# broadinstitute/Tangram

Hardware: NVIDIA H100
Metric: map_cells_to_space iterations/sec (higher is better)
Workload: dtype bf16 operands / f32 accumulate+state

## Files before the change

### tangram_b200/csrc/adam_rows.cuh

```cuda
#pragma once
#include "common.cuh"
#include "gemm_tc.cuh"

namespace tgb {

struct AdamRowsArgs {
  float* M; __nv_bfloat16* m; float* v;
  const __nv_bfloat16* dq;
  __nv_bfloat16* Pt;
  const RowConst* rowc;
  float* zsum; float* pxsum; float* l1sum; float* l2sum;
  int ld, V, row0, row1;
  float lam_r, lam_l1, lam_l2;
  AdamScalars a;
};

__device__ __forceinline__ void ldg256f(const float* src, float (&x)[8]) {
  asm volatile("ld.global.cs.v4.f32 {%0,%1,%2,%3}, [%8];\n\t"
               "ld.global.cs.v4.f32 {%4,%5,%6,%7}, [%8+16];"
               : "=f"(x[0]), "=f"(x[1]), "=f"(x[2]), "=f"(x[3]), "=f"(x[4]), "=f"(x[5]), "=f"(x[6]), "=f"(x[7]) : "l"(src));
}
__device__ __forceinline__ void stg256f(float* dst, const float (&x)[8]) {
  asm volatile("st.global.cs.v4.f32 [%0], {%1,%2,%3,%4};\n\t"
               "st.global.cs.v4.f32 [%0+16], {%5,%6,%7,%8};"
               ::"l"(dst), "f"(x[0]), "f"(x[1]), "f"(x[2]), "f"(x[3]), "f"(x[4]), "f"(x[5]), "f"(x[6]), "f"(x[7]) : "memory");
}
__device__ __forceinline__ uint4 ldg128_stream(const void* src) {
  uint4 r;
  asm volatile("ld.global.nc.L1::no_allocate.v4.b32 {%0,%1,%2,%3}, [%4];" : "=r"(r.x), "=r"(r.y), "=r"(r.z), "=r"(r.w) : "l"(src));
  return r;
}

struct AdamRowsLoad { float x[8], m[8], v[8]; uint4 d, mq; };

__device__ __forceinline__ void unpack_bf8(const uint4& q, float (&f)[8]) {
  const uint32_t w[4] = {q.x, q.y, q.z, q.w};
#pragma unroll
  for (int e = 0; e < 4; ++e) {
    const __nv_bfloat162 b = *reinterpret_cast<const __nv_bfloat162*>(&w[e]);
    f[2 * e] = __low2float(b); f[2 * e + 1] = __high2float(b);
  }
}
__device__ __forceinline__ uint4 pack_bf8(const float (&f)[8]) {
  uint4 o;
  __nv_bfloat162 b;
  b = __floats2bfloat162_rn(f[0], f[1]); o.x = *reinterpret_cast<uint32_t*>(&b);
  b = __floats2bfloat162_rn(f[2], f[3]); o.y = *reinterpret_cast<uint32_t*>(&b);
  b = __floats2bfloat162_rn(f[4], f[5]); o.z = *reinterpret_cast<uint32_t*>(&b);
  b = __floats2bfloat162_rn(f[6], f[7]); o.w = *reinterpret_cast<uint32_t*>(&b);
  return o;
}

#ifndef TGB_ADAM_MAXNREG
#define TGB_ADAM_MAXNREG 96
#endif
template <bool PLAIN>
__global__ void __maxnreg__(TGB_ADAM_MAXNREG)
k_adam_rows(const AdamRowsArgs p) {
  const int lane = threadIdx.x & 31;
  const int row = p.row0 + blockIdx.x * 8 + (threadIdx.x >> 5);
  if (row >= p.row1) return;
  const RowConst rc = p.rowc[row];
  const float lse_l2e = rc.lse * 1.4426950408889634f;
  const size_t base = (size_t)row * p.ld;
  float* Mr = p.M + base; __nv_bfloat16* mr = p.m + base; float* vr = p.v + base;
  const __nv_bfloat16* dr = p.dq + base;
  __nv_bfloat16* pr = p.Pt + base;

  const float k_nstep = -p.a.step_size;

  float zs = 0.f, pxs = 0.f, l1s = 0.f, l2s = 0.f;

  auto load = [&](int c, AdamRowsLoad& L) {
    ldg256f(Mr + c, L.x); L.mq = ldg128_stream(mr + c); ldg256f(vr + c, L.v);
    L.d = ldg128_stream(dr + c);
  };
  auto one = [&](float& x, float dq, float& m, float& v) -> float {
    const float pcur = fast_ex2(fmaf(x, 1.4426950408889634f, -lse_l2e));
    float g = dq - rc.r;
    if (p.lam_r != 0.f) g -= p.lam_r * ((x - rc.lse) - rc.h);
    g *= pcur;
    if (p.lam_l1 != 0.f) g += p.lam_l1 * (float)((x > 0.f) - (x < 0.f));
    if (p.lam_l2 != 0.f) g += 2.f * p.lam_l2 * x;
    m = fmaf(g - m, p.a.one_minus_beta1, m);
    v = fmaf(p.a.one_minus_beta2 * g, g, v * p.a.beta2);
    const float denom = fmaf(fast_sqrt(v), p.a.inv_bc2_sqrt, p.a.eps);
    x = fmaf(-p.a.step_size * m, fast_rcp(denom), x);
    const float pt = fast_ex2(fmaf(x, 1.4426950408889634f, -lse_l2e));
    zs += pt;
    if (p.pxsum) pxs = fmaf(pt, x, pxs);
    if (p.l1sum) { l1s += fabsf(x); l2s = fmaf(x, x, l2s); }
    return pt;
  };
  auto process = [&](int c, AdamRowsLoad& L) {
// ... 33 lines not shown
        const float dq = (e & 1) ? __high2float(d2) : __low2float(d2);
        pt[e] = (c + e < p.V) ? one(L.x[e], dq, L.m[e], L.v[e]) : 0.f;
      }
      stg256f(Mr + c, L.x); *reinterpret_cast<uint4*>(mr + c) = pack_bf8(L.m); stg256f(vr + c, L.v);
    } else {
#pragma unroll
      for (int e = 0; e < 8; ++e) pt[e] = 0.f;
    }
    *reinterpret_cast<uint4*>(pr + c) = pack_bf8(pt);
  };

  int c = lane * 8;
  for (; c + 256 < p.ld; c += 512) {
    AdamRowsLoad A, B;
    load(c, A);
    load(c + 256, B);
    process(c, A);
    process(c + 256, B);
  }
  if (c < p.ld) {
    AdamRowsLoad A;
    load(c, A);
    process(c, A);
  }
  zs = warp_sum(zs);
  if (p.pxsum) pxs = warp_sum(pxs);
  if (p.l1sum) { l1s = warp_sum(l1s); l2s = warp_sum(l2s); }
  if (lane == 0) {
    p.zsum[row] = zs;
    if (p.pxsum) p.pxsum[row] = pxs;
    if (p.l1sum) { p.l1sum[row] = l1s; p.l2sum[row] = l2s; }
  }
}

struct AdamRowsExactArgs {
  float* M; float* m; float* v;
  const float* dp;
  const RowStat* stats; const float* rdot;
  int ld, V, row0, row1;
  float lam_r, lam_l1, lam_l2;
  AdamScalars a;
};

__global__ void __launch_bounds__(256)
k_adam_rows_exact(const AdamRowsExactArgs p) {
  const int lane = threadIdx.x & 31;
  const int row = p.row0 + blockIdx.x * 8 + (threadIdx.x >> 5);
  if (row >= p.row1) return;
  const RowStat st = p.stats[row];
  const float r = p.rdot[row];
  const size_t base = (size_t)row * p.ld;
  float* Mr = p.M + base; float* mr = p.m + base; float* vr = p.v + base;
  const float* dr = p.dp + base;
  for (int c = lane * 8; c < p.V; c += 256) {
    float x[8], m[8], v[8], d[8];
    ldg256f(Mr + c, x); ldg256f(mr + c, m); ldg256f(vr + c, v); ldg256f(dr + c, d);
#pragma unroll
    for (int e = 0; e < 8; ++e) {
      if (c + e < p.V) {
        const float pr = softmax_prob(x[e], st);
        float g = d[e] - r;
        if (p.lam_r != 0.f) g -= p.lam_r * (((x[e] - st.mx) - st.log_z) - st.h);
        g *= pr;
        if (p.lam_l1 != 0.f) g += p.lam_l1 * (float)((x[e] > 0.f) - (x[e] < 0.f));
        if (p.lam_l2 != 0.f) g += 2.f * p.lam_l2 * x[e];
        x[e] = adam_update(x[e], g, m[e], v[e], p.a);
// ... 25 lines not shown
```

### tangram_b200/csrc/gemm_tc.cuh

```cuda
#pragma once
#include <cuda.h>
#include <cstdio>
#include "common.cuh"
#include "gemm_simt.cuh"

namespace tgb {

constexpr int TC_BM = 128;
constexpr int TC_BK = 64;
constexpr int TC_MMA_K = 16;
constexpr int TC_BN = 256;
constexpr int TC_THREADS = 384;
constexpr int TC_ACC = TC_BN / 2;

__device__ __forceinline__ uint32_t smem_u32(const void* p) { return (uint32_t)__cvta_generic_to_shared(p); }

__device__ __forceinline__ void mbar_init(uint64_t* bar, uint32_t count) {
  asm volatile("mbarrier.init.shared::cta.b64 [%0], %1;" ::"r"(smem_u32(bar)), "r"(count));
}
__device__ __forceinline__ void mbar_expect_tx(uint64_t* bar, uint32_t bytes) {
  asm volatile("mbarrier.arrive.expect_tx.shared::cta.b64 _, [%0], %1;" ::"r"(smem_u32(bar)), "r"(bytes) : "memory");
}
__device__ __forceinline__ void mbar_wait(uint64_t* bar, uint32_t parity) {
  asm volatile(
// ... 460 lines not shown
static inline int tc_init(TcContext& tc, char* err, size_t n) {
  void* fn = nullptr;
  cudaDriverEntryPointQueryResult qres;
  cudaError_t e = cudaGetDriverEntryPoint("cuTensorMapEncodeTiled", &fn, cudaEnableDefault, &qres);
  if (e != cudaSuccess || fn == nullptr || qres != cudaDriverEntryPointSuccess) {
    snprintf(err, n, "cuTensorMapEncodeTiled not available from the driver (%s)", cudaGetErrorString(e));
    return -2;
  }
  tc.encode = (PFN_encodeTiled)fn;
  int dev = 0;
  cudaGetDevice(&dev);
  cudaDeviceGetAttribute(&tc.num_sms, cudaDevAttrMultiProcessorCount, dev);
  return 0;
}

static inline int tc_make_map(TcContext& tc, CUtensorMap* map, const void* base, uint64_t cols, uint64_t rows,
                              uint64_t ld, uint32_t box_inner, uint32_t box_outer, char* err, size_t n) {
  cuuint64_t dims[2] = {cols, rows};
  cuuint64_t strides[1] = {ld * 2};
  cuuint32_t box[2] = {box_inner, box_outer};
  cuuint32_t estr[2] = {1, 1};
  CUresult r = tc.encode(map, CU_TENSOR_MAP_DATA_TYPE_BFLOAT16, 2, const_cast<void*>(base), dims, strides, box, estr,
                         CU_TENSOR_MAP_INTERLEAVE_NONE, CU_TENSOR_MAP_SWIZZLE_128B, CU_TENSOR_MAP_L2_PROMOTION_L2_256B,
                         CU_TENSOR_MAP_FLOAT_OOB_FILL_NONE);
  if (r != CUDA_SUCCESS) {
    snprintf(err, n, "cuTensorMapEncodeTiled failed (%d) cols=%llu rows=%llu ld=%llu box=%ux%u", (int)r,
             (unsigned long long)cols, (unsigned long long)rows, (unsigned long long)ld, box_inner, box_outer);
    return -2;
  }
  return 0;
}

template <class Kern, class... Args>
static inline int tc_launch(TcContext& tc, Kern kern, int smem, long long pairs, cudaStream_t s, const char* name, char* err,
                            size_t n, Args... args) {
  cudaLaunchAttribute attr[1];
  attr[0].id = cudaLaunchAttributeClusterDimension;
  attr[0].val.clusterDim.x = 2;
  attr[0].val.clusterDim.y = 1;
  attr[0].val.clusterDim.z = 1;
  cudaLaunchConfig_t cfg = {};
  cfg.blockDim = dim3(TC_THREADS);
  cfg.dynamicSmemBytes = (size_t)smem;
  cfg.stream = s;
  cfg.attrs = attr;
  cfg.numAttrs = 1;
  const void* key = reinterpret_cast<const void*>(kern);
  int slot = -1;
  for (int i = 0; i < 16; ++i) {
    if (tc.smem_fn[i] == key) { slot = i; break; }
    if (tc.smem_fn[i] == nullptr && slot < 0) slot = i;
  }
  if (slot < 0) { snprintf(err, n, "launch %s: more than 16 tensor-core kernels", name); return -2; }
  if (tc.smem_fn[slot] != key || tc.smem_bytes[slot] != smem) {
    cudaError_t e = cudaFuncSetAttribute(kern, cudaFuncAttributeMaxDynamicSharedMemorySize, smem);
    if (e != cudaSuccess) { snprintf(err, n, "cudaFuncSetAttribute(smem=%d): %s", smem, cudaGetErrorString(e)); return -2; }
    cfg.gridDim = dim3(2);
    int c = 0;
    e = cudaOccupancyMaxActiveClusters(&c, kern, &cfg);
    if (e != cudaSuccess || c < 1) {
      snprintf(err, n, "launch %s: no 2-CTA cluster with %d B of shared memory fits (%s)", name, smem, cudaGetErrorString(e));
      return -2;
    }
    tc.smem_fn[slot] = key; tc.smem_bytes[slot] = smem; tc.clusters[slot] = c;
  }
  cfg.gridDim = dim3((unsigned)(2 * (pairs < tc.clusters[slot] ? pairs : tc.clusters[slot])));
  cudaError_t e = cudaLaunchKernelEx(&cfg, kern, args...);
  if (e == cudaSuccess) e = cudaGetLastError();
  if (e != cudaSuccess) { snprintf(err, n, "launch %s: %s", name, cudaGetErrorString(e)); return -2; }
  return 0;
}

constexpr int TC_STAGE_BYTES = (TC_BM + TC_BN) * TC_BK * 2;
constexpr int TC_SMEM_LIMIT = 227 * 1024;
template <class Epi>
constexpr int tc_stages() {
  const int fit = (TC_SMEM_LIMIT - 2048 - Epi::kSmemBytes) / TC_STAGE_BYTES;
  return fit < 4 ? fit : 4;
}
template <class Epi>
constexpr int tc_smem() { return tc_stages<Epi>() * TC_STAGE_BYTES + Epi::kSmemBytes + 1024; }
constexpr int TC_SMEM = tc_smem<TcEpiStore>();
static inline int tc_dp_row_parts(int V) { return (int)ceil_div(V, TC_BN); }
static inline int tc_splits(int num_sms, long long tiles, long long k_total, int min_k) {
  long long s = (2LL * num_sms + tiles - 1) / tiles;
  const long long max_s = (k_total + min_k - 1) / min_k;
  if (s > max_s) s = max_s;
  if (s < 1) s = 1;
  const long long kps = ((k_total + s - 1) / s + TC_BK - 1) / TC_BK * TC_BK;
  return (int)((k_total + kps - 1) / kps);
}
static inline int tc_splits_for_chain(long long k_total, int max_chain) {
  long long s = (k_total + max_chain - 1) / max_chain;
  if (s < 1) s = 1;
  const long long kps = ((k_total + s - 1) / s + TC_BK - 1) / TC_BK * TC_BK;
  return (int)((k_total + kps - 1) / kps);
}
static inline int tc_forward_splits(int num_sms, int N, int V, int Ke) {
  return tc_splits(num_sms, (long long)ceil_div(V, TC_BM) * ceil_div(Ke, TC_BN), N, 512);
}
static inline int tc_kps(int k_total, int splits) {
  return (int)(round_up(ceil_div(k_total, splits), TC_BK));
}
static inline long long tc_pairs(int tiles_m, int tiles_n, int splits) { return (long long)(tiles_m + 1) / 2 * tiles_n * splits; }

static inline int tc_make_maps(TcContext& tc, TcMaps* maps, const __nv_bfloat16* base, size_t plane_elems, int n_planes,
                               uint64_t cols, uint64_t rows, uint64_t ld, uint32_t bi, uint32_t bo, char* err, size_t n) {
  for (int p = 0; p < 3; ++p) {
    const __nv_bfloat16* ptr = base + (size_t)(p < n_planes ? p : 0) * plane_elems;
    if (tc_make_map(tc, &maps->m[p], ptr, cols, rows, ld, bi, bo, err, n)) return -2;
  }
  return 0;
}

struct TcPlan {
  TcMaps a, b;
  CUtensorMap pt, dq;
  bool ready = false;
};

static inline int tc_forward_plan(TcContext& tc, TcPlan& pl, const __nv_bfloat16* P, size_t p_plane, const __nv_bfloat16* Sx,
                                  size_t s_plane, int planes, int N, int V, int Ke, int ld, char* err, size_t n) {
  if (tc_make_maps(tc, &pl.a, P, p_plane, planes, V, N, ld, 64, 64, err, n)) return -2;
  if (tc_make_maps(tc, &pl.b, Sx, s_plane, planes, Ke, N, Ke, 64, 64, err, n)) return -2;
  pl.ready = true;
  return 0;
}
static inline int tc_forward_launch(TcContext& tc, const TcPlan& pl, int n_pairs, float* out, int N, int V, int Ke, int splits,
                                    cudaStream_t s, char* err, size_t n) {
  auto kern = k_gemm_tc<false, false, tc_stages<TcEpiStore>(), TcEpiStore>;
  TcEpiStore epi{out, Ke, (size_t)V * Ke, V, 0};
  const int tm = (int)ceil_div(V, TC_BM), tn = (int)ceil_div(Ke, TC_BN);
  return tc_launch(tc, kern, TC_SMEM, tc_pairs(tm, tn, splits), s, "tc_gemm_fwd", err, n, pl.a, pl.b, n_pairs, N, tc_kps(N, splits),
                   tm, tn, splits, 1, kPolicyEvictNormal, kPolicyEvictNormal, 0, 0, epi);
}
static inline int tc_forward_launch_rows(TcContext& tc, const TcPlan& pl, int n_pairs, float* out, int accumulate, int row0, int row1,
                                         int V, int Ke, cudaStream_t s, char* err, size_t n) {
  auto kern = k_gemm_tc<false, false, tc_stages<TcEpiStore>(), TcEpiStore>;
  TcEpiStore epi{out, Ke, (size_t)V * Ke, V, accumulate};
  const int tm = (int)ceil_div(V, TC_BM), tn = (int)ceil_div(Ke, TC_BN);
  return tc_launch(tc, kern, TC_SMEM, tc_pairs(tm, tn, 1), s, "tc_gemm_fwd", err, n, pl.a, pl.b, n_pairs, row1,
                   (int)round_up(row1 - row0, TC_BK), tm, tn, 1, 1, kPolicyEvictNormal, kPolicyEvictNormal, 0, row0, epi);
}

static inline int tc_dpstore_plan(TcContext& tc, TcPlan& pl, const __nv_bfloat16* Sxb, size_t s_plane, const __nv_bfloat16* dYb,
                                  size_t dy_plane, int planes, int N, int V, int Ke, char* err, size_t n) {
  if (tc_make_maps(tc, &pl.a, Sxb, s_plane, planes, Ke, N, Ke, 64, TC_BM, err, n)) return -2;
  if (tc_make_maps(tc, &pl.b, dYb, dy_plane, planes, Ke, V, Ke, 64, TC_BN / 2, err, n)) return -2;
  pl.ready = true;
  return 0;
}
static inline int tc_dpstore_epi_plan(TcContext& tc, TcPlan& pl, const __nv_bfloat16* Pt, const __nv_bfloat16* dq, int N, int ld,
                                      char* err, size_t n) {
  if (tc_make_map(tc, &pl.pt, Pt, ld, N, ld, 64, 64, err, n)) return -2;
  return tc_make_map(tc, &pl.dq, dq, ld, N, ld, 64, 64, err, n);
}
template <class Epi>
static inline int tc_dpstore_launch(TcContext& tc, const TcPlan& pl, int n_pairs, const Epi& epi, int row0, int row1, int V, int Ke,
                                    cudaStream_t s, char* err, size_t n) {
  const int tn = (int)ceil_div(V, TC_BN);
  auto kern = k_gemm_tc<true, true, tc_stages<Epi>(), Epi>;
  constexpr int smem = tc_smem<Epi>();
  const int tm0 = row0 / TC_BM, tm = (int)ceil_div(row1, TC_BM) - tm0;
  return tc_launch(tc, kern, smem, tc_pairs(tm, tn, 1), s, "tc_gemm_bwd_dp", err, n, pl.a, pl.b, n_pairs, Ke, Ke, tm, tn, 1, 1,
                   kPolicyEvictNormal, kPolicyEvictLast, tm0, 0, epi);
}

}
```

### tangram_b200/csrc/tangram_b200.cu

```cuda
#include "../../include/tangram_b200.h"

#include <algorithm>
#include <cmath>
#include <cstdarg>
#include <cstdio>
#include <cstdlib>
#include <cstring>
#include <mutex>
#include <string>
#include <thread>
#include <vector>

#include "common.cuh"
#include "kernels_elem.cuh"
#include "gemm_simt.cuh"
#include "gemm_tc.cuh"
#include "adam_rows.cuh"
#include "legacy_rng.cuh"
#include "agreement.cuh"
#include "annotate.cuh"
#include "project.cuh"
#include "group_stats.cuh"
#include "mt19937_jump.h"
#include "nccl_dl.h"
// ... 97 lines not shown
  int fwd_splits = 1;
  DevBuf<float> Ypart;
  DevBuf<float> Y;
  DevBuf<float> dY;
  DevBuf<__nv_bfloat16> dYb;
  DevBuf<float> ngc, ngr, WG, nwg, AG, nag, sgnG, Z, Zg, H;
  DevBuf<float> colpart, colpart_nb, colpart_go, rowpart, ctpart;
  DevBuf<float> coefA, coefB, coefAn, coefBn, coefAg, coefBg, coefAr, coefBr, densg;
  CsrDev W, WT, F, FT, A, AT;
  int nchunk = 0, ncolchunk = 0, nredchunk = 0, n_ct_blocks = 0, loss_rows = 16;
  DevBuf<float> colfin;
  bool masked = false;
  int n_active = 0;
  DevBuf<float> gene_act;
  DevBuf<float> gw;
  int val_every = 0;
  int64_t val_epoch = 0;
  int64_t val_row = -1;
  bool tail_stale = false;
  DevBuf<float> val_coef, val_rowpart, val_hist;
  DevBuf<float> hist;
  int64_t hist_len = 0, hist_cap = 0;
  bool have_expr = false, have_density = false, have_ct = false, have_mapping = false;
  bool in_step = false;
  int64_t launches = 0;
  float legacy_stats[8] = {0};
  TcContext tc;
  TcPlan plan_fwd, plan_dp;
  DevBuf<__nv_bfloat16> dq;
  DevBuf<__nv_bfloat16> mb;
  DevBuf<float> rcenter;
  DevBuf<float> dpf;
  bool pipelined = false;
  bool host_state = false;
  int R = 0;
  int ring_rows = 0;
  DevBuf<float> Mh, mh, vh;
  DevBuf<__nv_bfloat16> mbh;
  DevBuf<float> rM[2], rm[2], rv[2];
  DevBuf<__nv_bfloat16> rmb[2];
  cudaStream_t cin = nullptr, cout = nullptr;
  cudaEvent_t ev_in[2] = {}, ev_comp[2] = {}, ev_free[2] = {}, ev_start = nullptr, ev_last = nullptr;
  bool ring_used = false;
  int nchunks = 1, chunk_row[9] = {0};
  cudaStream_t hi = nullptr, lo = nullptr, sf = nullptr;
  cudaEvent_t ev_fork = nullptr, ev_join_hi = nullptr, ev_join_lo = nullptr, ev_join_sf = nullptr, ev_loss = nullptr;
  cudaEvent_t ev_g[8] = {}, ev_a[8] = {}, ev_f[8] = {};
  bool a_valid = false;
  bool fwd_ahead = false;
  bool recording = false;
  std::vector<LaunchRecord> records;
  void drop_records(size_t from) {
    for (size_t i = from; i < records.size(); ++i) cudaEventDestroy(records[i].ev);
    records.resize(from);
  }
  void* comm = nullptr;
  bool comm_owned = false;
  int comm_rank = 0, comm_world = 1;
  bool y_nccl = false;
  void* y_reg = nullptr;
  void release_exchange_registration() {
    if (!y_nccl) return;
    char e[64];
    if (NcclApi* a = nccl_api(e, sizeof(e))) {
      if (y_reg && comm) a->CommDeregister(comm, y_reg);
      a->MemFree(Y.p);
// ... 275 lines not shown
  } else {
    A(h->Pf.alloc(nv));
  }
  A(h->Sx.alloc((size_t)h->N * h->Ke));
  A(h->G.alloc(vk));
  A(h->d.alloc(h->V)); A(h->dsrc.alloc(h->N));
  A(h->stats.alloc(h->N)); A(h->rowaux.alloc((size_t)2 * h->N)); A(h->rdot.alloc(h->N));
  int nc = 1;
  if (h->bf16) {
    nc = h->N >= 32768 ? 4 : (h->N >= 8192 ? 2 : 1);
    if (const char* e = getenv("TGB200_CHUNKS")) nc = atoi(e);
    if (nc < 1) nc = 1;
    if (nc > 8) nc = 8;
    if (h->constrained) nc = 1;
    while (nc > 1 && h->N / nc < 1024) --nc;
  }
  h->nchunks = nc;
  for (int c = 0; c <= nc; ++c) h->chunk_row[c] = c == nc ? h->N : (int)round_up((int64_t)c * h->N / nc, 256);
  if (h->nchunks > 1) {
    int lo_p = 0, hi_p = 0;
    cudaDeviceGetStreamPriorityRange(&lo_p, &hi_p);
    const int mid_p = hi_p < lo_p ? hi_p + 1 : lo_p;
    bool ok = cudaStreamCreateWithPriority(&h->hi, cudaStreamNonBlocking, hi_p) == cudaSuccess &&
              cudaStreamCreateWithPriority(&h->sf, cudaStreamNonBlocking, mid_p) == cudaSuccess &&
              cudaStreamCreateWithPriority(&h->lo, cudaStreamNonBlocking, lo_p) == cudaSuccess;
    cudaEvent_t* evs[5] = {&h->ev_fork, &h->ev_join_hi, &h->ev_join_lo, &h->ev_join_sf, &h->ev_loss};
    for (auto e : evs) ok = ok && cudaEventCreateWithFlags(e, cudaEventDisableTiming) == cudaSuccess;
    for (int c = 0; c < 8; ++c)
      ok = ok && cudaEventCreateWithFlags(&h->ev_g[c], cudaEventDisableTiming) == cudaSuccess &&
           cudaEventCreateWithFlags(&h->ev_a[c], cudaEventDisableTiming) == cudaSuccess &&
           cudaEventCreateWithFlags(&h->ev_f[c], cudaEventDisableTiming) == cudaSuccess;
    if (!ok) A(fail(TGB200_ERR_CUDA, "stream / event creation failed: %s", cudaGetErrorString(cudaGetLastError())));
    h->pipelined = ok;
  }
  h->tc.num_sms = prop.multiProcessorCount;
  if (h->nchunks > 1) {
    h->fwd_splits = 1;
  } else if (h->tcm) {
    h->fwd_splits = tc_forward_splits(h->tc.num_sms, h->N, h->V, h->Ke);
    if (h->x3) h->fwd_splits = std::max(h->fwd_splits, tc_splits_for_chain(h->N, 2048));
  } else {
    const int tiles = (int)(ceil_div(h->V, 128) * ceil_div(h->Ke, 128));
    h->fwd_splits = std::clamp((int)ceil_div(2 * h->tc.num_sms, tiles), 1, (int)ceil_div(h->N, 512));
  }
  if (h->fwd_splits > 1) A(h->Ypart.alloc((size_t)h->fwd_splits * vk));
  A(h->Y.alloc(vk + kTail));
  if (!h->tcm) A(h->dY.alloc(vk));
  if (h->constrained) {
    A(h->Fl.alloc(h->N)); A(h->mF.alloc(h->N)); A(h->vF.alloc(h->N)); A(h->fsig.alloc(h->N));
    A(h->Sf.alloc((size_t)h->N * h->Ke)); A(h->fscal.alloc(4));
  }
  h->r_parts = h->tcm ? tc_dp_row_parts(h->V) : (int)ceil_div(h->Ke, SG_BN);
  A(h->rpart.alloc((size_t)h->r_parts * h->N));
  A(h->ngc.alloc(h->Ke)); A(h->ngr.alloc(h->V));
  h->loss_rows = 16;
  while (ceil_div(h->V, h->loss_rows) > 512 && h->loss_rows < kLossRowsMax) h->loss_rows += 16;
  h->nchunk = (int)ceil_div(h->V, h->loss_rows);
  A(h->colfin.alloc((size_t)7 * h->Ke));
  h->ncolchunk = (int)ceil_div(h->Ke, kLossCols);
  h->nredchunk = (int)ceil_div(h->Ke, kLossColsBlk);
  A(h->colpart.alloc((size_t)h->nchunk * 3 * h->Ke));
  A(h->coefA.alloc(h->Ke)); A(h->coefB.alloc(h->Ke));
  A(h->gw.alloc(h->Ke));
  A(h->densg.alloc(h->V));
  if (cfg->lambda_g2 != 0.f) { A(h->rowpart.alloc((size_t)h->ncolchunk * h->V * 2)); A(h->coefAr.alloc(h->V)); A(h->coefBr.alloc(h->V)); }
  if (cfg->lambda_neighborhood_g1 > 0.f) {
// ... 731 lines not shown
  if (c.lambda_getis_ord > 0.f && !h->A.set) return fail(TGB200_ERR_STATE, "lambda_getis_ord > 0 needs the spatial_weights graph");
  if (h->constrained && !h->have_filter) return fail(TGB200_ERR_STATE, "constrained mode: call tgb200_set_filter first");
  return TGB200_OK;
}

struct Lanes { cudaStream_t caller, work, update, ahead; };
static Lanes lanes_of(const tgb200_mapper* h, cudaStream_t s) {
  return h->pipelined ? Lanes{s, h->hi, h->lo, h->sf} : Lanes{s, s, s, s};
}
static int fork_streams(tgb200_mapper* h, const Lanes& L) {
  if (L.work == L.caller) return TGB200_OK;
  CK(cudaEventRecord(h->ev_fork, L.caller));
  CK(cudaStreamWaitEvent(L.work, h->ev_fork, 0));
  return TGB200_OK;
}
static int join_streams(tgb200_mapper* h, const Lanes& L) {
  if (L.work == L.caller) return TGB200_OK;
  CK(cudaEventRecord(h->ev_join_hi, L.work));
  CK(cudaStreamWaitEvent(L.caller, h->ev_join_hi, 0));
  CK(cudaEventRecord(h->ev_join_lo, L.update));
  CK(cudaStreamWaitEvent(L.caller, h->ev_join_lo, 0));
  CK(cudaEventRecord(h->ev_join_sf, L.ahead));
  CK(cudaStreamWaitEvent(L.caller, h->ev_join_sf, 0));
  return TGB200_OK;
}

static int forward_plan(tgb200_mapper* h) {
  if (h->plan_fwd.ready) return TGB200_OK;
  const __nv_bfloat16* sB = h->bf16 ? h->Sxs.p : h->Sxb.p;
  return tc_forward_plan(h->tc, h->plan_fwd, h->Pb.p, (size_t)h->N * h->ld, sB, (size_t)h->N * h->Ke, h->x3 ? 3 : 1, h->N, h->V,
                         h->Ke, h->ld, g_err, sizeof(g_err));
}

static int forward_chunk(tgb200_mapper* h, cudaStream_t s, int c, int fresh, const float* lseA, float* lseT) {
  float* rowaux = needs_rowaux(h->cfg) ? h->rowaux.p : nullptr;
  CKS(forward_plan(h));
  const int r0 = h->chunk_row[c], r1 = h->chunk_row[c + 1];
  if (h->a_valid) CK(cudaStreamWaitEvent(s, h->ev_a[c], 0));
  k_row_norm<<<(unsigned)ceil_div(r1 - r0, 256), 256, 0, s>>>(fresh, h->zsum.p, h->pxsum.p, h->l1sum.p, h->l2sum.p,
                                                             lseA, lseT, h->inv_zt.p, h->stats.p, rowaux, r0, r1);
  LAUNCH_CHECK("row_norm");
  const long long nq = (long long)(r1 - r0) * (h->Ke / 4);
  k_scale_rows_bf16<<<(unsigned)ceil_div(nq, 256), 256, 0, s>>>(s_act(h), h->inv_zt.p, r0, r1, h->Ke, h->Sxs.p);
  LAUNCH_CHECK("scale_rows");
  if (h->nchunks > 1) {
    CKS(tc_forward_launch_rows(h->tc, h->plan_fwd, 1, h->Y.p, c > 0 ? 1 : 0, r0, r1, h->V, h->Ke, s, g_err, sizeof(g_err)));
    mark(h, s, "tc_gemm_fwd");
  }
  return TGB200_OK;
}

static int forward_pass(tgb200_mapper* h, cudaStream_t s, int want_entropy) {
  float* rowaux = needs_rowaux(h->cfg) ? h->rowaux.p : nullptr;
  if (h->bf16) {
    if (h->p_state == PState::stale) {
      CKS(launch_softmax_rows<__nv_bfloat16>(h, s, h->Pb.p, 1, rowaux));
      h->p_state = PState::fresh;
    }
    if (h->fwd_ahead) {
      h->fwd_ahead = false;
      for (int c = 0; c < h->nchunks; ++c) CK(cudaStreamWaitEvent(s, h->ev_f[c], 0));
    } else {
      for (int c = 0; c < h->nchunks; ++c) CKS(forward_chunk(h, s, c, h->p_state == PState::fresh ? 1 : 0, h->lseA, h->lseT));
    }
    if (h->nchunks > 1) return TGB200_OK;
  } else if (h->x3) {
    CKS(launch_softmax_rows<float>(h, s, (float*)nullptr, want_entropy, rowaux, Split3{h->Pb.p, (size_t)h->N * h->ld}));
  } else {
    CKS(launch_softmax_rows<float>(h, s, h->Pf.p, want_entropy, rowaux));
  }
  const size_t vk = (size_t)h->V * h->Ke;
  float* out = h->fwd_splits > 1 ? h->Ypart.p : h->Y.p;
  if (h->tcm) {
    CKS(forward_plan(h));
    CKS(tc_forward_launch(h->tc, h->plan_fwd, h->x3 ? 6 : 1, out, h->N, h->V, h->Ke, h->fwd_splits, s, g_err, sizeof(g_err)));
    mark(h, s, "tc_gemm_fwd");
  } else {
    GemmArgs g;
    g.A = h->Pf.p; g.lda = h->ld; g.B = s_act(h); g.ldb = h->Ke;
    g.M = h->V; g.N = h->Ke; g.K = h->N;
    g.k_per_split = (int)round_up(ceil_div(h->N, h->fwd_splits), 16);
    EpiStorePartial epi{out, h->Ke, vk};
    dim3 grid((unsigned)ceil_div(h->Ke, SG_BN), (unsigned)ceil_div(h->V, SG_BM), h->fwd_splits);
    k_gemm_simt<false, false, EpiStorePartial><<<grid, SG_THREADS, 0, s>>>(g, epi);
    LAUNCH_CHECK("simt_gemm_fwd");
  }
  return TGB200_OK;
}

static int sum_forward_planes(tgb200_mapper* h, cudaStream_t s) {
  if (h->cfg.n_cells_global == h->N || h->fwd_splits <= 1) return TGB200_OK;
  const size_t vk = (size_t)h->V * h->Ke;
  k_sum_planes<<<(unsigned)ceil_div(vk, 256), 256, 0, s>>>(h->Ypart.p, h->fwd_splits, vk, h->Y.p);
  LAUNCH_CHECK("sum_planes");
  return TGB200_OK;
}
// ... 128 lines not shown

static AdamScalars adam_scalars(const tgb200_config& c, int64_t t, float lr) {
  const double b1 = as_written(c.adam_beta1), b2 = as_written(c.adam_beta2);
  const double bc1 = 1.0 - std::pow(b1, (double)t), bc2 = 1.0 - std::pow(b2, (double)t);
  AdamScalars a;
  a.beta1 = c.adam_beta1; a.beta2 = c.adam_beta2;
  a.one_minus_beta1 = (float)(1.0 - b1); a.one_minus_beta2 = (float)(1.0 - b2);
  a.step_size = (float)(as_written(lr) / bc1);
  a.bc2_sqrt = (float)std::pow(bc2, 0.5);
  a.inv_bc2_sqrt = (float)(1.0 / std::pow(bc2, 0.5));
  a.eps = c.adam_eps;
  return a;
}

static int filter_update(tgb200_mapper* h, cudaStream_t s, const AdamScalars& a) {
  k_filter_update<<<(unsigned)ceil_div(h->N, 256), 256, 0, s>>>(h->N, h->rdot.p, h->fsig.p, h->fscal.p, h->cfg.lambda_count,
                                                                 h->cfg.lambda_f_reg, a, h->Fl.p, h->mF.p, h->vF.p);
  LAUNCH_CHECK("filter_update");
  return TGB200_OK;
}

static int backward_bf16(tgb200_mapper* h, const Lanes& L, const AdamScalars& a, bool next_forward) {
  if (!h->plan_dp.ready) {
    CKS(tc_dpstore_epi_plan(h->tc, h->plan_dp, h->Pb.p, h->dq.p, h->N, h->ld, g_err, sizeof(g_err)));
    CKS(tc_dpstore_plan(h->tc, h->plan_dp, h->Sxb.p, 0, h->dYb.p, 0, 1, h->N, h->V, h->Ke, g_err, sizeof(g_err)));
  }
  cudaStream_t s = L.work, su = L.update;
  const bool two_streams = su != s;
  const bool prefetch = two_streams && next_forward;
  if (prefetch) CK(cudaEventRecord(h->ev_loss, s));
  for (int c = 0; c < h->nchunks; ++c) {
    const int r0 = h->chunk_row[c], r1 = h->chunk_row[c + 1];
    TcEpiDpStore epi{h->plan_dp.pt, h->plan_dp.dq, h->ld, h->rcenter.p, h->rpart.p, h->N};
    CKS(tc_dpstore_launch(h->tc, h->plan_dp, 1, epi, r0, r1, h->V, h->Ke, s, g_err, sizeof(g_err)));
    mark(h, s, "tc_gemm_bwd_dp");
    if (two_streams) {
      CK(cudaEventRecord(h->ev_g[c], s));
      CK(cudaStreamWaitEvent(su, h->ev_g[c], 0));
    }
    k_rowdot_finalize_staged<<<(unsigned)ceil_div(r1 - r0, 256), 256, 0, su>>>(h->rpart.p, h->r_parts, h->N, r0, r1, h->lseT, h->inv_zt.p,
                                                                               h->stats.p, h->rcenter.p, h->rdot.p, h->rowc.p);
    { cudaStream_t s = su; LAUNCH_CHECK("rowdot_finalize"); }
    if (h->constrained) CKS(filter_update(h, su, a));
    CKS(staged_rows(h, su, r0, r1, true, [&](int b0, int b1, const StagedPtrs& sp) -> int {
      AdamRowsArgs ar{sp.M, sp.mb, sp.v, h->dq.p, h->Pb.p, reinterpret_cast<const RowConst*>(h->rowc.p),
                      h->zsum.p, h->pxsum.p, h->l1sum.p, h->l2sum.p, h->ld, h->V, b0, b1,
                      h->cfg.lambda_r, h->cfg.lambda_l1, h->cfg.lambda_l2, a};
      if (adam_rows_launch(ar, su)) return fail(TGB200_ERR_CUDA, "launch adam_rows: %s", cudaGetErrorString(cudaGetLastError()));
      mark(h, su, "adam_rows");
      return TGB200_OK;
    }));
    if (two_streams) CK(cudaEventRecord(h->ev_a[c], su));
    h->a_valid = two_streams;
    if (prefetch) {
      if (c == 0) CK(cudaStreamWaitEvent(L.ahead, h->ev_loss, 0));
      CKS(forward_chunk(h, L.ahead, c, 0, h->lseT, h->lseA));
      CK(cudaEventRecord(h->ev_f[c], L.ahead));
    }
  }
  h->fwd_ahead = prefetch;
  float* t = h->lseA; h->lseA = h->lseT; h->lseT = t;
  h->p_state = PState::updated;
  return TGB200_OK;
}

static int backward_bf16x3(tgb200_mapper* h, cudaStream_t s, const AdamScalars& a) {
  const size_t nkp = (size_t)h->N * h->Ke, vkp = (size_t)h->V * h->Ke, nvp = (size_t)h->N * h->ld;
  if (!h->plan_dp.ready)
    CKS(tc_dpstore_plan(h->tc, h->plan_dp, h->Sxb.p, nkp, h->dYb.p, vkp, 3, h->N, h->V, h->Ke, g_err, sizeof(g_err)));
  TcEpiDpStoreF32 epi{h->dpf.p, h->ld, h->Pb.p, nvp, h->rpart.p, h->N};
  CKS(tc_dpstore_launch(h->tc, h->plan_dp, 6, epi, 0, h->N, h->V, h->Ke, s, g_err, sizeof(g_err)));
  mark(h, s, "tc_gemm_bwd_dp");
  k_rowdot_finalize<<<(unsigned)ceil_div(h->N, 256), 256, 0, s>>>(h->rpart.p, h->r_parts, h->N, h->rdot.p);
  LAUNCH_CHECK("rowdot_finalize");
  if (h->constrained) CKS(filter_update(h, s, a));
  return staged_rows(h, s, 0, h->N, true, [&](int b0, int b1, const StagedPtrs& sp) -> int {
    AdamRowsExactArgs ar{sp.M, sp.m, sp.v, h->dpf.p, h->stats.p, h->rdot.p, h->ld, h->V, b0, b1,
                         h->cfg.lambda_r, h->cfg.lambda_l1, h->cfg.lambda_l2, a};
    if (adam_rows_exact_launch(ar, s)) return fail(TGB200_ERR_CUDA, "launch adam_rows_exact: %s", cudaGetErrorString(cudaGetLastError()));
    mark(h, s, "adam_rows");
    return TGB200_OK;
  });
}

static int backward_fp32(tgb200_mapper* h, cudaStream_t s, const AdamScalars& a) {
  GemmArgs g;
  g.A = h->Pf.p; g.lda = h->ld; g.B = h->dY.p; g.ldb = h->Ke;
  g.M = h->N; g.N = h->Ke; g.K = h->V; g.k_per_split = (int)round_up(h->V, 16);
  EpiRowDot epi_r{s_act(h), h->Ke, h->rpart.p};
  dim3 grid_r((unsigned)ceil_div(h->Ke, SG_BN), (unsigned)ceil_div(h->N, SG_BM), 1);
  k_gemm_simt<true, false, EpiRowDot><<<grid_r, SG_THREADS, 0, s>>>(g, epi_r);
  LAUNCH_CHECK("simt_gemm_rowdot");
  k_rowdot_finalize<<<(unsigned)ceil_div(h->N, 256), 256, 0, s>>>(h->rpart.p, h->r_parts, h->N, h->rdot.p);
  LAUNCH_CHECK("rowdot_finalize");
  if (h->constrained) CKS(filter_update(h, s, a));
  g.A = s_act(h); g.lda = h->Ke; g.B = h->dY.p; g.ldb = h->Ke;
  g.M = h->N; g.N = h->V; g.K = h->Ke; g.k_per_split = h->Ke;
  EpiAdam epi{h->M.p, h->m.p, h->v.p, h->ld, h->V, h->stats.p, h->rdot.p, h->cfg.lambda_r, h->cfg.lambda_l1, h->cfg.lambda_l2, a};
  dim3 grid((unsigned)ceil_div(h->V, SG_BN), (unsigned)ceil_div(h->N, SG_BM), 1);
  k_gemm_simt<true, true, EpiAdam><<<grid, SG_THREADS, 0, s>>>(g, epi);
  LAUNCH_CHECK("simt_gemm_bwd_adam");
  return TGB200_OK;
}

// ... 871 lines not shown
    } else {
      CK(cudaMemcpy2DAsync(Xf[k].p, sizeof(float) * ldx, X + r0 * x_ld, sizeof(float) * x_ld, sizeof(float) * n_genes, nb,
                           cudaMemcpyDefault, cp.s));
    }
    CK(cudaEventRecord(cp.copied[k], cp.s));
    return TGB200_OK;
  };
  CKS(stage(0));
  for (int64_t b = 0; b < n_blocks; ++b) {
    const int k = (int)(b & 1);
    const int64_t r0 = b * B, nb = std::min(B, rows - r0), nb64 = round_up(nb, 64);
    CK(cudaStreamWaitEvent(s, cp.copied[k], 0));
    const Split3 mp{Mp.p, (size_t)B * ldm};
    if (h) {
      CKS(launch_softmax_rows<float>(h, s, (float*)nullptr, 0, nullptr, mp, (int)r0, (int)nb));
    } else {
      const long long m4 = nb * ldm / 4;
      k_split3<<<(unsigned)ceil_div(m4, 256), 256, 0, s>>>(Mf[k].p, mp, m4);
      CK(cudaGetLastError());
    }
    if (nb < nb64)
      for (int p = 0; p < 3; ++p) CK(cudaMemsetAsync(Mp.p + ((size_t)p * B + nb) * ldm, 0, 2 * (nb64 - nb) * ldm, s));
    if (csr) {
      const CsrSplitArgs a{P[k].p, I[k].p, D[k].p, (int)nb, (int)nb64, (int)n_genes, (int)ldx, Split3{Xp.p, (size_t)B * ldx}, bad.p};
      k_csr_split3<<<(unsigned)ceil_div(nb64 * kWarp, kProjThreads), kProjThreads, 0, s>>>(a);
    } else {
      const long long x4 = nb64 * ldx / 4;
      k_split3<<<(unsigned)ceil_div(x4, 256), 256, 0, s>>>(Xf[k].p, Split3{Xp.p, (size_t)B * ldx}, x4);
    }
    CK(cudaGetLastError());
    CK(cudaEventRecord(cp.freed[k], s));
    for (int64_t c0 = 0; c0 < nb; c0 += kProjChain)
      CKS(tc_forward_launch_rows(tc, pl, 6, O.p, b > 0 || c0 > 0, (int)c0, (int)std::min(nb, c0 + kProjChain), (int)cols,
                                 (int)ldx, s, g_err, sizeof(g_err)));
    if (b + 1 < n_blocks) CKS(stage(b + 1));
  }
  int bad_host = 0;
  CK(cudaMemcpyAsync(&bad_host, bad.p, sizeof(int), cudaMemcpyDeviceToHost, s));
  CK(cudaStreamSynchronize(s));
  if (bad_host)
    return fail(TGB200_ERR_INVALID, "a CSR column index is outside [0, %lld) or not strictly increasing within its row",
                (long long)n_genes);
  CK(cudaMemcpy2DAsync(out, sizeof(float) * n_genes, O.p, sizeof(float) * ldx, sizeof(float) * n_genes, cols,
                       cudaMemcpyDefault, s));
  CK(cudaStreamSynchronize(s));
  return TGB200_OK;
}

extern "C" int tgb200_project_map(const float* map, int64_t rows, int64_t cols, int64_t ld, const float* X, int64_t x_ld,
                                  const int64_t* indptr, const int32_t* indices, const float* data, int64_t nnz,
                                  int64_t n_genes, float* out, int64_t block_rows, int32_t device, void* stream) {
  if (!map || !out) return fail(TGB200_ERR_INVALID, "null argument");
  return project_blocks(nullptr, map, rows, cols, ld, X, x_ld, indptr, indices, data, nnz, n_genes, out, block_rows, device,
                        (cudaStream_t)stream);
}

extern "C" int tgb200_project(tgb200_mapper* h, const float* X, int64_t n_cols, float* out, void* stream) {
  if (!h || !X || !out || n_cols <= 0) return fail(TGB200_ERR_INVALID, "bad argument");
  if (!h->have_mapping) return fail(TGB200_ERR_STATE, "no mapping set");
  return project_blocks(h, nullptr, h->N, h->V, h->ld, X, n_cols, nullptr, nullptr, nullptr, 0, n_cols, out, 0, h->cfg.device,
                        (cudaStream_t)stream);
}

namespace {
constexpr int64_t kGsBlocks = 8;
constexpr int64_t kGsMaxBlock = 32 * kGsRange;
}
// ... 210 lines not shown
    CK(cudaEventRecord(cp.freed[k], s));
    if (b + 1 < n_blocks) CKS(stage(b + 1));
  }
  int bad_host = 0;
  CK(cudaMemcpyAsync(&bad_host, bad.p, sizeof(int), cudaMemcpyDeviceToHost, s));
  CK(cudaStreamSynchronize(s));
  if (bad_host)
    return fail(TGB200_ERR_INVALID, "a CSR column index is outside [0, %lld) or not strictly increasing within its row",
                (long long)n_genes);
  CK(cudaMemcpyAsync(sum_out, sum.p, sizeof(double) * T * G, cudaMemcpyDefault, s));
  CK(cudaMemcpyAsync(sumsq_out, sq.p, sizeof(double) * T * G, cudaMemcpyDefault, s));
  if (nnz_out) CK(cudaMemcpyAsync(nnz_out, cntd.p, sizeof(int64_t) * T * G, cudaMemcpyDefault, s));
  CK(cudaStreamSynchronize(s));
  return TGB200_OK;
}

extern "C" int tgb200_group_stats(const float* X, int64_t x_ld, const int64_t* indptr, const int32_t* indices,
                                  const float* data, int64_t nnz, int64_t rows, int64_t n_genes,
                                  const int32_t* labels, int32_t n_labels, double* sum_out, double* sumsq_out,
                                  int64_t* nnz_out, int64_t block_rows, int32_t device, void* stream) {
  return group_stats_pass(GsValue::kIdentity, 1.0, X, x_ld, indptr, indices, data, nnz, rows, n_genes, labels, n_labels,
                          sum_out, sumsq_out, nnz_out, block_rows, device, stream);
}

extern "C" int tgb200_group_stats_expm1(const float* X, int64_t x_ld, const int64_t* indptr, const int32_t* indices,
                                        const float* data, int64_t nnz, int64_t rows, int64_t n_genes,
                                        const int32_t* labels, int32_t n_labels, double* sum_out, double* sumsq_out,
                                        int64_t* nnz_out, int64_t block_rows, int32_t device, void* stream,
                                        double scale) {
  if (!std::isfinite(scale)) return fail(TGB200_ERR_INVALID, "scale=%g is not finite", scale);
  return group_stats_pass(GsValue::kExpm1, scale, X, x_ld, indptr, indices, data, nnz, rows, n_genes, labels, n_labels,
                          sum_out, sumsq_out, nnz_out, block_rows, device, stream);
}
```

Baseline: 46.75.

## Reserve SMs in pipelined GEMM launches so the Adam update overlaps on the other stream

Adds a keep_sms parameter to tc_launch that shrinks the persistent GEMM grid by that many SMs (rounded to clusters). In the two-stream pipelined path, the backward dp GEMM for chunks after the first and the prefetched forward GEMM (except the last chunk) leave 16 SMs free by default (overridable via TGB200_UPDATE_SMS), so the concurrent Adam row-update kernel can run alongside instead of waiting for GEMM CTAs to drain. Also refactors the Adam kernel body into a device function and adds a compile-time-guarded overlap probe for timing. The cost is fewer SMs for the GEMM while it runs.

```diff
diff --git a/tangram_b200/csrc/adam_rows.cuh b/tangram_b200/csrc/adam_rows.cuh
--- a/tangram_b200/csrc/adam_rows.cuh
+++ b/tangram_b200/csrc/adam_rows.cuh
@@ -55,11 +55,7 @@
 #define TGB_ADAM_MAXNREG 96
 #endif
 template <bool PLAIN>
-__global__ void __maxnreg__(TGB_ADAM_MAXNREG)
-k_adam_rows(const AdamRowsArgs p) {
-  const int lane = threadIdx.x & 31;
-  const int row = p.row0 + blockIdx.x * 8 + (threadIdx.x >> 5);
-  if (row >= p.row1) return;
+__device__ __forceinline__ void adam_row(const AdamRowsArgs& p, int row, int lane) {
   const RowConst rc = p.rowc[row];
   const float lse_l2e = rc.lse * 1.4426950408889634f;
   const size_t base = (size_t)row * p.ld;
@@ -159,6 +155,21 @@
     if (p.l1sum) { p.l1sum[row] = l1s; p.l2sum[row] = l2s; }
   }
 }
+template <bool PLAIN>
+__global__ void __maxnreg__(TGB_ADAM_MAXNREG)
+k_adam_rows(const AdamRowsArgs p) {
+  const int row = p.row0 + blockIdx.x * 8 + (threadIdx.x >> 5);
+  if (row < p.row1) adam_row<PLAIN>(p, row, threadIdx.x & 31);
+}
+#ifdef TGB_OVERLAP_PROBE
+template <bool PLAIN>
+__global__ void __maxnreg__(TGB_ADAM_MAXNREG)
+k_adam_rows_probe(const AdamRowsArgs p) {
+  const int warps = blockDim.x >> 5;
+  for (int row = p.row0 + blockIdx.x * warps + (threadIdx.x >> 5); row < p.row1; row += gridDim.x * warps)
+    adam_row<PLAIN>(p, row, threadIdx.x & 31);
+}
+#endif
 
 struct AdamRowsExactArgs {
   float* M; float* m; float* v;
diff --git a/tangram_b200/csrc/gemm_tc.cuh b/tangram_b200/csrc/gemm_tc.cuh
--- a/tangram_b200/csrc/gemm_tc.cuh
+++ b/tangram_b200/csrc/gemm_tc.cuh
@@ -516,8 +516,8 @@
 }
 
 template <class Kern, class... Args>
-static inline int tc_launch(TcContext& tc, Kern kern, int smem, long long pairs, cudaStream_t s, const char* name, char* err,
-                            size_t n, Args... args) {
+static inline int tc_launch(TcContext& tc, Kern kern, int smem, long long pairs, int keep_sms, cudaStream_t s, const char* name,
+                            char* err, size_t n, Args... args) {
   cudaLaunchAttribute attr[1];
   attr[0].id = cudaLaunchAttributeClusterDimension;
   attr[0].val.clusterDim.x = 2;
@@ -548,7 +548,8 @@
     }
     tc.smem_fn[slot] = key; tc.smem_bytes[slot] = smem; tc.clusters[slot] = c;
   }
-  cfg.gridDim = dim3((unsigned)(2 * (pairs < tc.clusters[slot] ? pairs : tc.clusters[slot])));
+  const int clusters = std::max(1, tc.clusters[slot] - (keep_sms + 1) / 2);
+  cfg.gridDim = dim3((unsigned)(2 * (pairs < clusters ? pairs : clusters)));
   cudaError_t e = cudaLaunchKernelEx(&cfg, kern, args...);
   if (e == cudaSuccess) e = cudaGetLastError();
   if (e != cudaSuccess) { snprintf(err, n, "launch %s: %s", name, cudaGetErrorString(e)); return -2; }
@@ -615,15 +616,15 @@
   auto kern = k_gemm_tc<false, false, tc_stages<TcEpiStore>(), TcEpiStore>;
   TcEpiStore epi{out, Ke, (size_t)V * Ke, V, 0};
   const int tm = (int)ceil_div(V, TC_BM), tn = (int)ceil_div(Ke, TC_BN);
-  return tc_launch(tc, kern, TC_SMEM, tc_pairs(tm, tn, splits), s, "tc_gemm_fwd", err, n, pl.a, pl.b, n_pairs, N, tc_kps(N, splits),
+  return tc_launch(tc, kern, TC_SMEM, tc_pairs(tm, tn, splits), 0, s, "tc_gemm_fwd", err, n, pl.a, pl.b, n_pairs, N, tc_kps(N, splits),
                    tm, tn, splits, 1, kPolicyEvictNormal, kPolicyEvictNormal, 0, 0, epi);
 }
 static inline int tc_forward_launch_rows(TcContext& tc, const TcPlan& pl, int n_pairs, float* out, int accumulate, int row0, int row1,
-                                         int V, int Ke, cudaStream_t s, char* err, size_t n) {
+                                         int V, int Ke, int keep_sms, cudaStream_t s, char* err, size_t n) {
   auto kern = k_gemm_tc<false, false, tc_stages<TcEpiStore>(), TcEpiStore>;
   TcEpiStore epi{out, Ke, (size_t)V * Ke, V, accumulate};
   const int tm = (int)ceil_div(V, TC_BM), tn = (int)ceil_div(Ke, TC_BN);
-  return tc_launch(tc, kern, TC_SMEM, tc_pairs(tm, tn, 1), s, "tc_gemm_fwd", err, n, pl.a, pl.b, n_pairs, row1,
+  return tc_launch(tc, kern, TC_SMEM, tc_pairs(tm, tn, 1), keep_sms, s, "tc_gemm_fwd", err, n, pl.a, pl.b, n_pairs, row1,
                    (int)round_up(row1 - row0, TC_BK), tm, tn, 1, 1, kPolicyEvictNormal, kPolicyEvictNormal, 0, row0, epi);
 }
 
@@ -641,12 +642,12 @@
 }
 template <class Epi>
 static inline int tc_dpstore_launch(TcContext& tc, const TcPlan& pl, int n_pairs, const Epi& epi, int row0, int row1, int V, int Ke,
-                                    cudaStream_t s, char* err, size_t n) {
+                                    int keep_sms, cudaStream_t s, char* err, size_t n) {
   const int tn = (int)ceil_div(V, TC_BN);
   auto kern = k_gemm_tc<true, true, tc_stages<Epi>(), Epi>;
   constexpr int smem = tc_smem<Epi>();
   const int tm0 = row0 / TC_BM, tm = (int)ceil_div(row1, TC_BM) - tm0;
-  return tc_launch(tc, kern, smem, tc_pairs(tm, tn, 1), s, "tc_gemm_bwd_dp", err, n, pl.a, pl.b, n_pairs, Ke, Ke, tm, tn, 1, 1,
+  return tc_launch(tc, kern, smem, tc_pairs(tm, tn, 1), keep_sms, s, "tc_gemm_bwd_dp", err, n, pl.a, pl.b, n_pairs, Ke, Ke, tm, tn, 1, 1,
                    kPolicyEvictNormal, kPolicyEvictLast, tm0, 0, epi);
 }
 
diff --git a/tangram_b200/csrc/tangram_b200.cu b/tangram_b200/csrc/tangram_b200.cu
--- a/tangram_b200/csrc/tangram_b200.cu
+++ b/tangram_b200/csrc/tangram_b200.cu
@@ -153,6 +153,7 @@
   DevBuf<float> rcenter;
   DevBuf<float> dpf;
   bool pipelined = false;
+  int update_sms = 0;
   bool host_state = false;
   int R = 0;
   int ring_rows = 0;
@@ -494,6 +495,8 @@
            cudaEventCreateWithFlags(&h->ev_f[c], cudaEventDisableTiming) == cudaSuccess;
     if (!ok) A(fail(TGB200_ERR_CUDA, "stream / event creation failed: %s", cudaGetErrorString(cudaGetLastError())));
     h->pipelined = ok;
+    h->update_sms = 16;
+    if (const char* e = getenv("TGB200_UPDATE_SMS")) h->update_sms = std::max(0, atoi(e));
   }
   h->tc.num_sms = prop.multiProcessorCount;
   if (h->nchunks > 1) {
@@ -1291,7 +1294,7 @@
                          h->Ke, h->ld, g_err, sizeof(g_err));
 }
 
-static int forward_chunk(tgb200_mapper* h, cudaStream_t s, int c, int fresh, const float* lseA, float* lseT) {
+static int forward_chunk(tgb200_mapper* h, cudaStream_t s, int c, int fresh, const float* lseA, float* lseT, int keep_sms) {
   float* rowaux = needs_rowaux(h->cfg) ? h->rowaux.p : nullptr;
   CKS(forward_plan(h));
   const int r0 = h->chunk_row[c], r1 = h->chunk_row[c + 1];
@@ -1303,7 +1306,7 @@
   k_scale_rows_bf16<<<(unsigned)ceil_div(nq, 256), 256, 0, s>>>(s_act(h), h->inv_zt.p, r0, r1, h->Ke, h->Sxs.p);
   LAUNCH_CHECK("scale_rows");
   if (h->nchunks > 1) {
-    CKS(tc_forward_launch_rows(h->tc, h->plan_fwd, 1, h->Y.p, c > 0 ? 1 : 0, r0, r1, h->V, h->Ke, s, g_err, sizeof(g_err)));
+    CKS(tc_forward_launch_rows(h->tc, h->plan_fwd, 1, h->Y.p, c > 0 ? 1 : 0, r0, r1, h->V, h->Ke, keep_sms, s, g_err, sizeof(g_err)));
     mark(h, s, "tc_gemm_fwd");
   }
   return TGB200_OK;
@@ -1320,7 +1323,7 @@
       h->fwd_ahead = false;
       for (int c = 0; c < h->nchunks; ++c) CK(cudaStreamWaitEvent(s, h->ev_f[c], 0));
     } else {
-      for (int c = 0; c < h->nchunks; ++c) CKS(forward_chunk(h, s, c, h->p_state == PState::fresh ? 1 : 0, h->lseA, h->lseT));
+      for (int c = 0; c < h->nchunks; ++c) CKS(forward_chunk(h, s, c, h->p_state == PState::fresh ? 1 : 0, h->lseA, h->lseT, 0));
     }
     if (h->nchunks > 1) return TGB200_OK;
   } else if (h->x3) {
@@ -1515,7 +1518,8 @@
   for (int c = 0; c < h->nchunks; ++c) {
     const int r0 = h->chunk_row[c], r1 = h->chunk_row[c + 1];
     TcEpiDpStore epi{h->plan_dp.pt, h->plan_dp.dq, h->ld, h->rcenter.p, h->rpart.p, h->N};
-    CKS(tc_dpstore_launch(h->tc, h->plan_dp, 1, epi, r0, r1, h->V, h->Ke, s, g_err, sizeof(g_err)));
+    CKS(tc_dpstore_launch(h->tc, h->plan_dp, 1, epi, r0, r1, h->V, h->Ke, two_streams && c > 0 ? h->update_sms : 0, s, g_err,
+                          sizeof(g_err)));
     mark(h, s, "tc_gemm_bwd_dp");
     if (two_streams) {
       CK(cudaEventRecord(h->ev_g[c], s));
@@ -1537,7 +1541,7 @@
     h->a_valid = two_streams;
     if (prefetch) {
       if (c == 0) CK(cudaStreamWaitEvent(L.ahead, h->ev_loss, 0));
-      CKS(forward_chunk(h, L.ahead, c, 0, h->lseT, h->lseA));
+      CKS(forward_chunk(h, L.ahead, c, 0, h->lseT, h->lseA, c + 1 < h->nchunks ? h->update_sms : 0));
       CK(cudaEventRecord(h->ev_f[c], L.ahead));
     }
   }
@@ -1552,7 +1556,7 @@
   if (!h->plan_dp.ready)
     CKS(tc_dpstore_plan(h->tc, h->plan_dp, h->Sxb.p, nkp, h->dYb.p, vkp, 3, h->N, h->V, h->Ke, g_err, sizeof(g_err)));
   TcEpiDpStoreF32 epi{h->dpf.p, h->ld, h->Pb.p, nvp, h->rpart.p, h->N};
-  CKS(tc_dpstore_launch(h->tc, h->plan_dp, 6, epi, 0, h->N, h->V, h->Ke, s, g_err, sizeof(g_err)));
+  CKS(tc_dpstore_launch(h->tc, h->plan_dp, 6, epi, 0, h->N, h->V, h->Ke, 0, s, g_err, sizeof(g_err)));
   mark(h, s, "tc_gemm_bwd_dp");
   k_rowdot_finalize<<<(unsigned)ceil_div(h->N, 256), 256, 0, s>>>(h->rpart.p, h->r_parts, h->N, h->rdot.p);
   LAUNCH_CHECK("rowdot_finalize");
@@ -2490,7 +2494,7 @@
     CK(cudaEventRecord(cp.freed[k], s));
     for (int64_t c0 = 0; c0 < nb; c0 += kProjChain)
       CKS(tc_forward_launch_rows(tc, pl, 6, O.p, b > 0 || c0 > 0, (int)c0, (int)std::min(nb, c0 + kProjChain), (int)cols,
-                                 (int)ldx, s, g_err, sizeof(g_err)));
+                                 (int)ldx, 0, s, g_err, sizeof(g_err)));
     if (b + 1 < n_blocks) CKS(stage(b + 1));
   }
   int bad_host = 0;
@@ -2767,3 +2771,54 @@
   return group_stats_pass(GsValue::kExpm1, scale, X, x_ld, indptr, indices, data, nnz, rows, n_genes, labels, n_labels,
                           sum_out, sumsq_out, nnz_out, block_rows, device, stream);
 }
+
+#ifdef TGB_OVERLAP_PROBE
+extern "C" TGB200_API int tgb200_debug_overlap_probe(tgb200_mapper* h, int32_t kind, int32_t cap, int32_t update_ctas,
+                                                     int32_t what, int32_t reps, float* out) {
+  if (!h || !out || reps < 1 || what < 1 || what > 3) return fail(TGB200_ERR_INVALID, "bad argument");
+  if (!h->bf16 || !h->pipelined || h->host_state || !h->plan_dp.ready || !h->plan_fwd.ready)
+    return fail(TGB200_ERR_STATE, "needs a resident, pipelined bf16 handle that has run an iteration");
+  CK(cudaSetDevice(h->cfg.device));
+  const int c0 = h->chunk_row[0], c1 = h->chunk_row[1], c2 = h->chunk_row[2];
+  const AdamScalars a = adam_scalars(h->cfg, h->step > 0 ? h->step : 1, 0.1f);
+  const AdamRowsArgs ar{h->M.p, h->mb.p, h->v.p, h->dq.p, h->Pb.p, reinterpret_cast<const RowConst*>(h->rowc.p),
+                        h->zsum.p, h->pxsum.p, h->l1sum.p, h->l2sum.p, h->ld, h->V, c0, c1,
+                        h->cfg.lambda_r, h->cfg.lambda_l1, h->cfg.lambda_l2, a};
+  const bool plain = ar.lam_r == 0.f && ar.lam_l1 == 0.f && ar.lam_l2 == 0.f;
+  const int keep = cap > 0 ? std::max(0, h->tc.num_sms - 2 * cap) : 0;
+  cudaEvent_t ev[4];
+  for (auto& e : ev) CK(cudaEventCreate(&e));
+  int st = TGB200_OK;
+  CK(cudaDeviceSynchronize());
+  for (int r = 0; r < reps && st == TGB200_OK; ++r) {
+    CK(cudaEventRecord(ev[0], h->hi));
+    CK(cudaStreamWaitEvent(h->lo, ev[0], 0));
+    if (what & 1) {
+      if (kind == 0) {
+        TcEpiDpStore epi{h->plan_dp.pt, h->plan_dp.dq, h->ld, h->rcenter.p, h->rpart.p, h->N};
+        st = tc_dpstore_launch(h->tc, h->plan_dp, 1, epi, c1, c2, h->V, h->Ke, keep, h->hi, g_err, sizeof(g_err));
+      } else {
+        st = tc_forward_launch_rows(h->tc, h->plan_fwd, 1, h->Y.p, 1, c1, c2, h->V, h->Ke, keep, h->hi, g_err, sizeof(g_err));
+      }
+    }
+    if (what & 2) {
+      if (update_ctas <= 0) {
+        if (adam_rows_launch(ar, h->lo)) st = fail(TGB200_ERR_CUDA, "launch adam_rows");
+      } else if (plain) {
+        k_adam_rows_probe<true><<<update_ctas, 512, 0, h->lo>>>(ar);
+      } else {
+        k_adam_rows_probe<false><<<update_ctas, 512, 0, h->lo>>>(ar);
+      }
+      if (cudaGetLastError() != cudaSuccess) st = fail(TGB200_ERR_CUDA, "launch adam_rows_probe");
+    }
+    CK(cudaEventRecord(ev[1], h->hi));
+    CK(cudaEventRecord(ev[2], h->lo));
+    CK(cudaStreamWaitEvent(h->hi, ev[2], 0));
+    CK(cudaEventRecord(ev[3], h->hi));
+    CK(cudaEventSynchronize(ev[3]));
+    for (int i = 0; i < 3; ++i) CK(cudaEventElapsedTime(&out[3 * r + i], ev[0], ev[i + 1]));
+  }
+  for (auto& e : ev) cudaEventDestroy(e);
+  return st;
+}
+#endif
```

Result: faster. 48.83, median of 6 (+4.5%).
